# NickDrake117/GNNkeras

Measured on AMD Instinct MI355X. Metric: node-state updates/s (arcs x iterations / s), forward Loop, higher is better.
Workload: dtype f32; 1 GPU; C4 Erdos-Renyi 1000000 nodes / 10000000 arcs, state_dim=64, max_iteration=50, threshold=0 (k=50), node-focused, average aggregation, BN+Dense(159->64,selu) state net

## Files before the change

### gnnkeras_amd/_native.py

```python
from __future__ import annotations

import ctypes as C
import os
import subprocess

import torch

HERE = os.path.dirname(os.path.abspath(__file__))
CSRC = os.path.join(HERE, 'csrc')
LIB_PATH = os.environ.get('GNNKERAS_AMD_LIB') or os.path.join(CSRC, 'libgnnloop.so')

GNN_ABI_VERSION = 10
GNN_MAX_LAYERS = 8
GNN_MAX_TYPES = 8

ACTIVATIONS = {'linear': 0, None: 0, 'relu': 1, 'selu': 2, 'tanh': 3, 'sigmoid': 4, 'elu': 5, 'softplus': 6,
               'softmax': 7}
FOCUS = {'n': 0, 'a': 1, 'g': 2}
FLAG_UNFUSED = 1
FLAG_NO_EARLY_EXIT = 2
FLAG_FUSED_GEN_MASK = 7 << 4
FLAG_TRAIN_HIDDEN_SMALL = 1 << 8
XC_FILL, XC_VALID = 0, 1
FLAG_LDS_HIDDEN = 1 << 9
FLAG_FUSED_GEN2, FLAG_FUSED_GEN4, FLAG_FUSED_GEN5, FLAG_FUSED_GEN6, FLAG_FUSED_GEN7 = 2 << 4, 4 << 4, 5 << 4, 6 << 4, 7 << 4

EXPORTS = ['gnn_last_error', 'gnn_last_status', 'gnn_last_kernel_name', 'gnn_abi_version', 'gnn_struct_size', 'gnn_loop_workspace_bytes', 'gnn_loop_forward', 'gnn_loop_groups_supported', 'gnn_loop_group_max_nodes', 'gnn_aggregate',
           'gnn_loop_xc_applies', 'gnn_loop_route_name', 'gnn_train_xc_applies',
           'gnn_mlp_workspace_bytes', 'gnn_mlp_forward', 'gnn_converged', 'gnn_state_step', 'gnn_state_step_agg', 'gnn_state_ld', 'gnn_debug_occupy', 'gnn_debug_occupy_until', 'gnn_debug_expiry_beacon', 'gnn_debug_host_flag',
           'gnn_debug_f4_tile_plan', 'gnn_debug_f4_tile_queue_const', 'gnn_debug_f4_last_tickets',
           'gnn_device_malloc', 'gnn_device_free', 'gnn_ipc_export', 'gnn_ipc_open', 'gnn_ipc_close', 'gnn_shard_iteration_peers', 'gnn_peer_wait', 'gnn_peer_publish', 'gnn_shard_iteration_split_rows',
           'gnn_shard_setup', 'gnn_shard_iteration', 'gnn_shard_output', 'gnn_gather_rows',
           'gnn_shard_can_split', 'gnn_shard_partial', 'gnn_shard_iteration_split',
           'gnn_dense', 'gnn_fold_bn', 'gnn_dense_grad_workspace_bytes', 'gnn_dense_grad', 'gnn_act_grad',
           'gnn_colstats_workspace_bytes', 'gnn_colstats', 'gnn_first_layer_param_grads', 'gnn_bn_input_grad',
           'gnn_scatter_add_rows', 'gnn_axpby', 'gnn_loss_grad', 'gnn_dropout', 'gnn_adam_step', 'gnn_adam_multi', 'gnn_sgd_step',
           'gnn_converged_gated', 'gnn_aggregate_gated', 'gnn_train_workspace_bytes', 'gnn_train_step', 'gnn_train_groups_supported', 'gnn_ragged_copy',
           'gnn_train_step_ex', 'gnn_train_phases_supported', 'gnn_gate_all',
           'gnn_train_step_composite_ex', 'gnn_train_composite_phases_supported', 'gnn_train_composite_phase_scratch_bytes',
           'gnn_comm_unique_id', 'gnn_comm_create', 'gnn_comm_destroy', 'gnn_shard_loop']
GNN_MAX_SEGMENTS = 6
LOSSES = {'categorical_crossentropy': 0, 'cce': 0, 'binary_crossentropy': 1, 'bce': 1, 'mse': 2,
          'mean_squared_error': 2, 'mae': 3, 'mean_absolute_error': 3}

_f32p = C.POINTER(C.c_float)
# ... 205 lines not shown
        l.gnn_shard_iteration_peers.restype = C.c_int
        l.gnn_shard_iteration_peers.argtypes = [C.POINTER(LoopArgs), C.c_void_p, C.c_void_p, C.c_int32, C.c_void_p, C.c_int32, C.c_int32, C.c_void_p, C.c_int32,
                                                C.POINTER(PeerSet)]
        l.gnn_peer_wait.restype = C.c_int
        l.gnn_peer_wait.argtypes = [C.c_void_p, C.c_int32, C.c_int32, C.c_int32, C.c_void_p, C.c_void_p]
        l.gnn_peer_publish.restype = C.c_int
        l.gnn_peer_publish.argtypes = [C.POINTER(PeerSet), C.c_void_p, C.c_void_p, C.c_int64, C.c_int32, C.c_int32, C.c_int32, C.c_void_p]
        l.gnn_debug_host_flag.restype = C.c_int
        l.gnn_debug_host_flag.argtypes = [C.POINTER(C.POINTER(C.c_int32)), C.POINTER(C.c_void_p)]
        l.gnn_debug_f4_tile_plan.restype = None
        l.gnn_debug_f4_tile_plan.argtypes = [C.c_int32, C.c_int32, C.c_int32, C.POINTER(C.c_int32)]
        l.gnn_debug_f4_tile_queue_const.restype = C.c_int32
        l.gnn_debug_f4_tile_queue_const.argtypes = [C.c_int32, C.c_int32]
        l.gnn_debug_f4_last_tickets.restype = C.c_longlong
        l.gnn_debug_f4_last_tickets.argtypes = []
        l.gnn_debug_expiry_beacon.restype = C.c_int
        l.gnn_debug_expiry_beacon.argtypes = [C.POINTER(C.c_void_p), C.c_int32, C.c_void_p]
        l.gnn_state_step_agg.restype = C.c_int
        l.gnn_state_step_agg.argtypes = [C.POINTER(LoopArgs), C.c_void_p, C.c_void_p, C.c_int32, C.c_void_p, C.c_int32, C.c_void_p, C.c_void_p]
        l.gnn_state_ld.restype = C.c_int32
        l.gnn_state_ld.argtypes = [C.c_int32]
        l.gnn_shard_setup.restype = C.c_int
        l.gnn_shard_setup.argtypes = [C.POINTER(LoopArgs)]
        l.gnn_shard_iteration.restype = C.c_int
        l.gnn_shard_iteration.argtypes = [C.POINTER(LoopArgs), C.c_void_p, C.c_void_p, C.c_int32, C.c_void_p, C.c_int32,
                                          C.c_int32, C.c_void_p, C.c_int32]
        l.gnn_shard_output.restype = C.c_int
        l.gnn_shard_output.argtypes = [C.POINTER(LoopArgs), C.c_void_p, C.c_void_p, C.c_int32]
        vp, i32, f32, sz = C.c_void_p, C.c_int32, C.c_float, C.c_size_t
        protos = {
# ... 88 lines not shown
```

### gnnkeras_amd/csrc/gnnloop.hip

```cpp
#include <hip/hip_runtime.h>
#include <stdarg.h>
#include <stddef.h>
#include <stdio.h>
#include <stdlib.h>
#include <string.h>
#include <algorithm>
#include <mutex>
#include <string>
#include <vector>

#include "../../include/gnnloop.h"
#include "kernels_general.hpp"
#include "kernel_state_fused2.hpp"
#include "kernel_state_fused4.hpp"
#include "kernel_state_small.hpp"
#include "kernel_state_mid.hpp"
#include "kernel_state_lds.hpp"
#include "kernel_state_lds_types.hpp"
#include "kernel_state_wide.hpp"
#include "kernels_batch.hpp"
#include "kernels_setup.hpp"
#include "kernel_rowdense.hpp"
#include "kernel_state_xwide.hpp"

// ... 38 lines not shown
    if (S <= 128) {
        int p = 16;
        while (p < S) p <<= 1;
        return p;
    }
    return round_up(S, 4);
}

struct Knobs {
    int pin;
    int flag_pin, env_pin;
    int mid_max_nodes;
    bool prefix_fusion, xwide, rowdense;
    bool xc; int xc_min_nodes;
    bool tile_queue;
};
const Knobs &process_knobs() {
    static const Knobs once = [] {
        Knobs k = {};
        const char *e;
        k.env_pin = (e = getenv("GNN_FUSED_KERNEL")) ? atoi(e) : 0;
        k.mid_max_nodes = (e = getenv("GNN_MID_MAX_NODES")) ? atoi(e) : 36000;
        k.prefix_fusion = !((e = getenv("GNN_PREFIX_FUSION")) && e[0] == '0');
        k.xwide = !((e = getenv("GNN_XWIDE")) && atoi(e) == 0);
        k.rowdense = !((e = getenv("GNN_ROWDENSE")) && e[0] == '0');
        return k;
    }();
    return once;
}
Knobs knobs(int flags) {
    Knobs k = process_knobs();
    k.flag_pin = (flags & GNN_FLAG_FUSED_GEN_MASK) >> 4;
    k.pin = k.flag_pin ? k.flag_pin : k.env_pin;
    const char *e = getenv("GNN_XC"), *m = getenv("GNN_XC_MIN_NODES");
    k.xc = !(e && atoi(e) == 0);
    k.xc_min_nodes = m ? atoi(m) : 196608;
    const char *q = getenv("GNN_F4_TILE_QUEUE");
    k.tile_queue = !(q && atoi(q) == 0);
    return k;
}

struct Carver {
    char *base;
    size_t off = 0;
    explicit Carver(void *b) : base((char *)b) {}
    template <typename T>
    T *take(size_t count) {
        off = (off + 255) & ~(size_t)255;
        T *p = base ? (T *)(base + off) : nullptr;
        off += count * sizeof(T);
        return p;
    }
};
// ... 334 lines not shown
    float *C; int ldC;
    float *Xc;
    float *Wx;
    bool xc_ok;
    float *buf[2], *agg;
    float *hid[2]; int ld_hid;
    float *Wf_out, *bf_out;
    float *ohid[2]; int ld_ohid;
    float *out_nodes;
    int *idx_src, *idx_dst;
    size_t bytes;
};

constexpr int GNN_SMALL_MAX_TILES = 512;
constexpr int GNN_LOOP_WORDS = 16 + 32 + gnn::MID_BAR_WORDS;
constexpr int GNN_TQ_WORDS = 8;
inline size_t tq_words(const gnn_loop_args_t &a) { return (size_t)GNN_TQ_WORDS * (size_t)a.max_iteration; }

int state_width(const gnn_loop_args_t &a) { return a.state_dim > 0 ? a.state_dim : a.dim_node_label; }

int make_plan(const gnn_loop_args_t &a, void *ws, Plan &p, bool validate_ptrs) {
    memset(&p, 0, sizeof(p));
    if (a.abi_version != GNN_ABI_VERSION) return fail("abi_version %d != %d", a.abi_version, GNN_ABI_VERSION);
    if (a.n_nodes < 0 || a.n_arcs < 0) return fail("negative graph size");
    if (a.state_dim < 0 || a.max_iteration < 0 || !(a.state_threshold >= 0.0f)) return fail("state_dim, max_iteration, state_threshold must be >= 0");
    p.composite = a.composite != 0;
    p.T = p.composite ? a.n_types : 1;
    if (p.T < 1 || p.T > GNN_MAX_TYPES) return fail("n_types %d out of [1,%d]", p.T, GNN_MAX_TYPES);
    if (p.composite && a.max_iteration < 1) return not_covered("composite GNN requires max_iteration > 0");
    p.N = a.n_nodes; p.E = a.n_arcs; p.L = a.dim_node_label; p.A = a.dim_arc_label;
    p.S = state_width(a);
    if (p.S < 1) return fail("state width is 0 (state_dim == 0 and dim_node_label == 0)");
// ... 77 lines not shown
        if (a.n_heavy_segments > 0) {
            if (!a.heavy_seg_beg || !a.heavy_seg_end) return fail("heavy_seg_beg / heavy_seg_end is NULL");
            TRY(check_csr(a.adjacency_light, "adjacency_light", p.N, (a.nodes_src ? a.adjacency.n_src : p.N) + a.n_heavy_segments));
        }
        if (p.composite) {
            if (!a.type_nodes && p.N > 0) return fail("type_nodes is NULL");
            if (a.type_offsets[0] != 0 || a.type_offsets[p.T] != p.N) return fail("type_offsets must span [0, n_nodes]");
            for (int t = 0; t < p.T; ++t)
                TRY(check_csr(a.composite_adjacency[t], "composite_adjacency", p.N, a.nodes_src ? a.adjacency.n_src : p.N));
        }
    }

    Carver c(ws);
    p.flags = c.take<int>(a.max_iteration + GNN_LOOP_WORDS + tq_words(a));
    p.err = p.flags ? p.flags + a.max_iteration + 12 : nullptr;
    p.tq = p.flags ? p.flags + a.max_iteration + GNN_LOOP_WORDS : nullptr;
    p.mid_bar = p.flags ? p.flags + ((a.max_iteration + 16 + 31) & ~31) : nullptr;
    p.pred0 = c.take<int>(std::max(GNN_SMALL_MAX_TILES, p.group_tiles));
    p.d_group_tabs = c.take<int>(a.n_groups > 0 ? 4 * ((size_t)a.n_groups + 1) : 0);
    p.set_bar = c.take<unsigned long long>(a.n_groups > 0 ? 2 * (size_t)a.n_groups : 0);
    for (int t = 0; t < p.T; ++t) {
        p.tp[t].Wf = c.take<float>((size_t)a.net_state[t].in_dim * a.net_state[t].units[0]);
        p.tp[t].bf = c.take<float>(a.net_state[t].units[0]);
    }
    p.Wf_out = c.take<float>((size_t)a.net_output.in_dim * a.net_output.units[0]);
    p.bf_out = c.take<float>(a.net_output.units[0]);
    p.agg_arcs = c.take<float>((size_t)p.N * std::max(p.A, 1));
    p.ld_agg_nodes = p.composite ? sum_dt : (a.state_dim > 0 ? p.L : 0);
    p.agg_nodes = c.take<float>((size_t)p.N * std::max(p.ld_agg_nodes, 1));
    p.ldC = (p.H1max + 3) & ~3;
    p.C = c.take<float>((size_t)p.N * p.ldC);
// ... 202 lines not shown
    sa.nodes_src = a.nodes_src ? a.nodes_src : a.nodes; sa.ld_nodes_src = a.nodes_src ? a.ld_nodes_src : a.ld_nodes;
    sa.adj = gnn::SetupCsr{a.adjacency.rowptr, a.adjacency.src, a.adjacency.w, a.adjacency.row_scale};
    sa.arc_labels = a.arc_labels; sa.ld_arcs = a.ld_arcs; sa.A = p.A;
    sa.arcnode = gnn::SetupCsr{a.arcnode.rowptr, a.arcnode.src, a.arcnode.w, a.arcnode.row_scale};
    if (a.state_dim > 0) { sa.row_nodes = p.S; sa.row_aggn = 2 * p.S + p.L; sa.row_agga = 2 * p.S + 2 * p.L; }
    else                 { sa.row_agga = 2 * p.S; }
    sa.C = p.C; sa.ldC = p.ldC;
    sa.state0 = a.state_dim > 0 ? a.state0 : a.nodes; sa.ld_s0 = a.state_dim > 0 ? p.S : a.ld_nodes;
    sa.S = p.S; sa.thr = a.state_threshold; sa.pred0 = p.pred0;
    sa.zero_a = p.flags; sa.n_a = a.max_iteration + GNN_LOOP_WORDS; sa.zero_b = a.k_out; sa.n_b = std::max(1, p.n_groups);
    gnn::k_setup_small<<<sa.n_tiles + 1, 256, gnn::setup_small_lds(sa.net.H, 2 * L + p.A, std::max(a.net_state[0].in_dim, a.net_output.in_dim)), st>>>(sa);
    LAUNCH_OK();
    return 0;
}

__device__ long long g_f4_last_tickets;
__global__ void k_fold_error(const int *err, float *k_out, const int *tq, int n_tq) {
    long long s = 0;
    for (int i = threadIdx.x; i < n_tq; i += 64) s += tq[i];
    for (int off = 32; off >= 1; off >>= 1) s += __shfl_xor(s, off, 64);
    if (threadIdx.x == 0) {
        g_f4_last_tickets = s;
        if (*err != 0) *k_out = -1.0e9f;
    }
}

int launch_fold_error(const Plan &p, float *k_out, hipStream_t st, const int *tq = nullptr, int n_tq = 0) {
    if (!k_out || !p.err) return 0;
    k_fold_error<<<1, 64, 0, st>>>(p.err, k_out, tq, n_tq);
    LAUNCH_OK();
    return 0;
}

__global__ void k_arc_endpoints(const int *__restrict__ out_index, const int *__restrict__ arc_src,
                                const int *__restrict__ arc_dst, int M, int *__restrict__ idx_src, int *__restrict__ idx_dst) {
    const int m = blockIdx.x * blockDim.x + threadIdx.x;
    if (m < M) { const int e = out_index[m]; idx_src[m] = arc_src[e]; idx_dst[m] = arc_dst[e]; }
}

int output_stage(const gnn_loop_args_t &a, const Plan &p, hipStream_t st) {
    if (p.M == 0) return 0;
    const bool with_labels = !p.composite && a.state_dim > 0;
    MlpRun r;
    r.mlp = &a.net_output; r.Wf = p.Wf_out; r.bf = p.bf_out;
// ... 71 lines not shown
    r.nseg = 1;
    r.segs[0] = gnn::Seg{p.agg, nullptr, p.SP, (int)m.units[1], 0};
    r.M = p.N;
    r.hid[0] = p.hid[0]; r.hid[1] = p.hid[1]; r.ld_hid = p.ld_hid;
    r.Y = dst; r.ldy = p.SP;
    r.gate = gate;
    if (flag_next) { r.pred_old = src; r.ld_pred = p.SP; r.pred_thr = a.state_threshold; r.pred_flag = flag_next; r.pred_k = k_out; r.pred_kval = k_val; }
    TRY(run_mlp(r, st));
    if (flag_next && !r.pred_fused) TRY(launch_converge(gate, dst, src, p.N, p.S, p.SP, p.SP, a.state_threshold, flag_next, k_out, k_val, st));
    return 0;
}

int iteration_fused(const gnn_loop_args_t &a, const Plan &p, IterKernel kernel, const int *gate, int n_gate, int gate_stride,
                    const float *src, float *dst, int row_base, int *flag_next, float *k_out, float k_val,
                    hipStream_t st, const gnn_csr_t *adj_override = nullptr, const float *agg_init = nullptr,
                    const int *rows_override = nullptr, int count_override = 0, const gnn_peer_set_t *peers = nullptr, int *tile_ctr = nullptr) {
    TRY(launch_heavy(a, p, n_gate == 1 ? gate : nullptr, src, st));
    const gnn_csr_t &adj = adj_override ? *adj_override : iter_adjacency(a, p);
    gnn::Fused2Args fa;
    memset(&fa, 0, sizeof(fa));
    fill_fused_args(fa, a, p, adj);
    fa.gate = n_gate ? gate : nullptr; fa.n_gate = n_gate; fa.gate_stride = gate_stride;
    fa.state_in = src; fa.state_out = dst; fa.row_base = row_base; fa.err = p.err;
    if (rows_override && fa.n_types == 1) {
        fa.tp[0].rows = rows_override; fa.tp[0].count = count_override;
        if (count_override == 0) fa.n_types = 0;
    }
    fa.flag_next = flag_next;
    fa.k_out = k_out; fa.k_val = k_val;
    fa.agg_init = agg_init;
    if (peers) {
        if (peers->n_peers < 0 || peers->n_peers > GNN_MAX_PEERS) return fail("n_peers %d out of [0, %d]", peers->n_peers, GNN_MAX_PEERS);
        fa.n_peers = peers->n_peers;
        for (int i = 0; i < peers->n_peers; ++i) fa.peer_out[i] = peers->state_out_full[i];
    }
    if (p.xc_ok && !adj.w && (agg_init || size_generation(p, a.flags) == 4)) fa.Xc = p.Xc;
    if (tile_ctr && kernel == IterKernel::fused4 && p.T == 1 && fa.n_types == 1 && !rows_override && !agg_init && !peers) fa.tq_ctr = tile_ctr;
    if (fa.n_types == 0) {
        if (k_out) TRY(launch_converge(fa.gate, src, src, 0, p.S, p.SP, p.SP, a.state_threshold, flag_next, k_out, k_val, st));
        return 0;
    }
    if (fa.n_peers > 0 && (p.SP == 128 || p.T != 1 || adj.w || a.net_state[0].n_layers != 1 || (p.SP != 32 && p.SP != 64) || p.n_heavy != 0))
        return fail("peer stores: homogeneous one-layer shards without per-arc weights or hub rows, state widths 17 .. 64");
    if (kernel == IterKernel::wide) FUSED_OK(gnn::launch_wide(fa, device_cus(), st, 0));
    else if (kernel == IterKernel::fused4 || agg_init || fa.n_peers > 0) FUSED_OK(gnn::launch_fused4(fa, p.SP, device_cus(), st));
    else FUSED_OK(gnn::launch_fused2(fa, p.SP, 8, device_cus(), st));
    return 0;
}

int loop_whole(const gnn_loop_args_t &a, const Plan &p, bool mid, const float *first, float *const B[2], const int *pred0,
               int n_pred0, float *state_final, hipStream_t st) {
    gnn::SmallArgs sa;
// ... 261 lines not shown
    if (first == a.state0 && a.state_out != a.state0 && (reinterpret_cast<uintptr_t>(a.state_out) & 15) == 0 && a.max_iteration > 0)
        B[a.max_iteration & 1] = a.state_out;
    if (a.ev_loop_begin) HIP_OK(hipEventRecord((hipEvent_t)a.ev_loop_begin, st));
    int persistent = 2;
    if (route.whole == WholeLoop::small) {
        persistent = loop_whole(a, p, false, first, B, small_setup ? p.pred0 : nullptr, small_setup ? p.group_tiles : 0, a.state_out, st);
        if (persistent == 1) return 1;
        if (persistent == 2 && small_setup) return fail("whole-loop kernel refused a graph its set-up kernel accepted");
    }
    bool loop_done = persistent == 0;
    if (!loop_done && route.try_mid) {
        const int rc = loop_whole(a, p, true, first, B, nullptr, 0, nullptr, st);
        if (rc == 1) return 1;
        loop_done = rc == 0;
    }
    int *const tq = (!small_setup && knobs(a.flags).tile_queue) ? p.tq : nullptr;
    for (int it = 0; !loop_done && it < a.max_iteration; ++it) {
        const int *gate = no_exit ? nullptr : p.flags + it;
        const float *src = it == 0 ? first : B[it & 1];
        float *dst = B[(it + 1) & 1];
        if (route.iter.fused())                  TRY(iteration_fused(a, p, kernel, gate, gate ? 1 : 0, 0, src, dst, 0, p.flags + it + 1, a.k_out, (float)(it + 1), st,
                                                                     nullptr, nullptr, nullptr, 0, nullptr, tq ? tq + (size_t)GNN_TQ_WORDS * it : nullptr));
        else if (kernel == IterKernel::prefix)   TRY(iteration_prefix(a, p, gate, src, dst, p.flags + it + 1, a.k_out, (float)(it + 1), st));
        else if (kernel == IterKernel::xwide)    TRY(iteration_xwide(a, p, gate, src, dst, p.flags + it + 1, a.k_out, (float)(it + 1), st));
        else                                     TRY(iteration_unfused(a, p, gate, src, dst, 0, p.flags + it + 1, a.k_out, (float)(it + 1), st));
    }

    if (a.ev_loop_end) HIP_OK(hipEventRecord((hipEvent_t)a.ev_loop_end, st));

    if (persistent != 0) {
        const long total = (long)p.N * p.S;
        if (total > 0) {
            gnn::k_select_state<<<std::min(cdiv(total, 256), 256 * 16), 256, 0, st>>>(a.k_out, first, B[0], B[1], p.SP, a.state_out, p.S, p.N, p.S);
            LAUNCH_OK();
        }
    }
    TRY(output_stage(a, p, st));
    if (!loop_done && (route.iter.fused() || kernel == IterKernel::xwide) && a.max_iteration > 0)
        TRY(launch_fold_error(p, a.k_out, st, tq, tq ? (int)tq_words(a) : 0));
    return 0;
}

int gnn_loop_groups_supported(const gnn_loop_args_t *args) {
    if (!args || args->n_groups < 1) return 0;
    Plan p;
    if (make_plan(*args, nullptr, p, false)) return 0;
    const LoopRoute route = route_loop(*args, p);
    if (route.whole == WholeLoop::lds || route.whole == WholeLoop::lds_types) return 2;
    if (p.composite || args->n_groups > GNN_MAX_GROUPS) return 0;
    return route.whole == WholeLoop::small && route.small_setup ? 1 : 0;
}

int gnn_loop_group_max_nodes(const gnn_loop_args_t *args) {
    if (!args) return 0;
// ... 120 lines not shown
    int polls = 0;
    while (wall_clock64() - t0 < ticks) {
        if (release && __hip_atomic_load(release, __ATOMIC_RELAXED, __HIP_MEMORY_SCOPE_SYSTEM) != 0) break;
        __builtin_amdgcn_s_sleep(64); ++polls;
    }
    if (threadIdx.x == 0 && polls < 0) { occ_smem[0] = polls; *sink = occ_smem[0]; }
}

void gnn_debug_f4_tile_plan(int32_t ntiles, int32_t n_workgroups, int32_t ahead, int32_t *out56) {
    for (int xcd = 0; xcd < 8; ++xcd) {
        const gnn::F4TilePlan q = gnn::f4_tile_plan(ntiles, n_workgroups, xcd, ahead);
        int32_t *o = out56 + 7 * xcd;
        o[0] = q.t_begin; o[1] = q.t_end; o[2] = q.blk; o[3] = q.T1; o[4] = q.pool_begin; o[5] = q.pool_end; o[6] = q.n_chunks;
    }
}
int32_t gnn_debug_f4_tile_queue_const(int32_t which, int32_t padded_width) {
    switch (which) {
        case 0: return gnn::F4_TQ_CH;
        case 1: return padded_width == 64 ? gnn::Fused4Cfg<64>::AHEAD : padded_width == 32 ? gnn::Fused4Cfg<32>::AHEAD : padded_width == 16 ? gnn::Fused4Cfg<16>::AHEAD : -1;
        case 2: return gnn::F4_TQ_MIN_SHARE;
        case 3: return gnn::F4_TQ_MAX_CHUNKS;
        case 4: return gnn::F4_TQ_TAB;
        default: return -1;
    }
}
long long gnn_debug_f4_last_tickets(void) {
    long long v = -1;
    if (hipDeviceSynchronize() != hipSuccess) return -1;
    return hipMemcpyFromSymbol(&v, HIP_SYMBOL(g_f4_last_tickets), sizeof(v)) == hipSuccess ? v : -1;
}
// ... 292 lines not shown
```

### gnnkeras_amd/csrc/kernel_state_fused2.hpp

```cpp
#pragma once
#include <hip/hip_runtime.h>
#include "kernels_general.hpp"

namespace gnn {

struct FusedType {
    const int *rows;
    int count;
    const float *Wf;
    int wrow_state, wrow_agg;
    int H, act;
    const float *W2;
    const float *b2;
    int act2;
    const float *Wc;
    int out2;
};

struct Fused2Args {
    const int *gate; int n_gate, gate_stride;
    const int *rowptr, *src;
    const float *w, *row_scale;
    const float *state_in;
    float *state_out;
    int row_base;
    const float *C; int ldC;
    int n_types;
    FusedType tp[GNN_MAX_TYPES];
    int blk_begin[GNN_MAX_TYPES + 1];
    int S;
    float thr;
    int *flag_next;
    float *k_out; float k_val;
    int *err;
    int *tq_ctr;
    const float *Xc;
    const float *agg_init;
    const void *hdr; void *hdr_write;
    float *peer_out[GNN_MAX_PEERS]; int n_peers;
};

inline char *last_kernel_name() { static thread_local char name[96] = ""; return name; }
#define GNN_SET_KERNEL_NAME(...) snprintf(::gnn::last_kernel_name(), 96, __VA_ARGS__)

template <int SP, int TM, int NW>
struct Fused2Cfg {
    static constexpr int NT = 64 * NW;
    static constexpr int LPR = SP / 4;
    static constexpr int NPP = NT / LPR;
    static constexpr int NPASS = TM / NPP;
// ... 323 lines not shown
```

### gnnkeras_amd/csrc/kernel_state_fused4.hpp

```cpp
#pragma once
#include <hip/hip_runtime.h>
#include "kernel_state_fused2.hpp"
#include "buffer_ops.hpp"

namespace gnn {

constexpr int XC_K = 32;

constexpr int F4_TQ_CH = 2;
constexpr int F4_TQ_NUM = 7, F4_TQ_DEN = 8;
constexpr int F4_TQ_TAB = 1024;
constexpr int F4_TQ_MAX_CHUNKS = 960;
constexpr int F4_TQ_MIN_SHARE = 16;
constexpr int F4_TQ_END = -2;
struct F4TilePlan { int t_begin, t_end, blk, T1, pool_begin, pool_end, n_chunks; };
__host__ __device__ inline F4TilePlan f4_tile_plan(int ntiles, int nblk, int xcd, int ahead) {
    F4TilePlan q;
    const int tpx = (ntiles + 7) >> 3;
    q.blk = (nblk + 7 - xcd) >> 3;
    q.t_begin = xcd * tpx < ntiles ? xcd * tpx : ntiles;
    q.t_end = (xcd + 1) * tpx < ntiles ? (xcd + 1) * tpx : ntiles;
    const int n = q.t_end - q.t_begin, b = q.blk > 0 ? q.blk : 1;
    const int n_min = ntiles - 7 * tpx > 0 ? ntiles - 7 * tpx : 0, b_max = (nblk + 7) >> 3;
    const bool queue = (nblk & 7) == 0 && nblk > 0 && n_min >= F4_TQ_MIN_SHARE * b_max && (int)((long)F4_TQ_NUM * n_min / ((long)F4_TQ_DEN * b_max)) >= ahead;
    if (!queue) {
        q.T1 = (n + b - 1) / b; q.pool_begin = q.pool_end = q.t_end; q.n_chunks = 0;
        return q;
    }
    q.T1 = (int)((long)F4_TQ_NUM * n / ((long)F4_TQ_DEN * b));
    if (n - q.T1 * b > F4_TQ_MAX_CHUNKS * F4_TQ_CH) q.T1 = (n - F4_TQ_MAX_CHUNKS * F4_TQ_CH + b - 1) / b;
    q.pool_begin = q.t_begin + q.T1 * b; q.pool_end = q.t_end;
    q.n_chunks = (q.pool_end - q.pool_begin + F4_TQ_CH - 1) / F4_TQ_CH;
    return q;
}

template <int SP, int NC = 4, bool L2 = false, bool XC = false, int VPL = 1, bool TQ = false>
struct Fused4Cfg {
    static constexpr int NW = 16, NT = 64 * NW;
    static constexpr int NCONS = NC;
    static constexpr int NPROD = NW - NCONS;
    static constexpr int LPR = SP / (4 * VPL);
    static constexpr int RPWV = 64 / LPR;
    static constexpr int PPT = 16 / RPWV;
    static constexpr int IPL = 16 / LPR;
    static constexpr int LDX = 2 * SP + 2;
    static constexpr bool SWZ = SP >= 32;
    static constexpr int LDW = SWZ ? SP : SP + 32;
    static constexpr int NCT = SP / 16;
    static constexpr int NS = SP == 64 ? (L2 ? 3 : (XC ? 4 : 5)) : 8;
    static constexpr int WROWS = 2 * SP + (XC ? XC_K : 0);
    static constexpr int SLOT = 16 * LDX;
    static constexpr int W2F = L2 ? SP * LDW + SP : 0;
    static constexpr int AHEAD = (2 * NPROD + PPT - 1) / PPT + F4_TQ_CH + 2;
    static constexpr size_t LDS_BYTES = sizeof(float) * ((size_t)NS * SLOT + WROWS * LDW + W2F) + sizeof(int) * (2 * NS + (TQ ? F4_TQ_TAB : 0));
};

__device__ __forceinline__ void activate4(int act, f32x4 &x) {
#define F4_ALL(expr)                                        \
    _Pragma("unroll") for (int e = 0; e < 4; ++e) {         \
        const float v = x[e];                               \
        x[e] = (expr);                                      \
    }
    switch (act) {
        case GNN_ACT_RELU: F4_ALL(fmaxf(v, 0.0f)) break;
        case GNN_ACT_SELU: F4_ALL(v > 0.0f ? 1.0507009873554805f * v : (1.0507009873554805f * 1.6732632423543772f) * (expf(v) - 1.0f)) break;
        case GNN_ACT_TANH: F4_ALL(tanhf(v)) break;
        case GNN_ACT_SIGMOID: F4_ALL(1.0f / (1.0f + expf(-v))) break;
        case GNN_ACT_ELU: F4_ALL(v > 0.0f ? v : expf(v) - 1.0f) break;
        case GNN_ACT_SOFTPLUS: F4_ALL(v > 20.0f ? v : log1pf(expf(v))) break;
// ... 44 lines not shown
    const int tid = threadIdx.x, lane = tid & 63, wave = tid >> 6;
    if (tid == 0) F4_STAMP(0);
    const int S = a.S;
    int ty = 0;
    while (ty + 1 < a.n_types && (int)blockIdx.x >= a.blk_begin[ty + 1]) ++ty;
    const FusedType tp = a.tp[ty];
    const int O2 = tp.out2 > 0 ? tp.out2 : S;
    const int bid = blockIdx.x - a.blk_begin[ty], nblk = a.blk_begin[ty + 1] - a.blk_begin[ty];
    const int count = tp.count;
    const int *__restrict__ rows = tp.rows;

    const int ntiles = (count + 15) / 16;
    const int xcd = bid & 7, lb = bid >> 3;
    const int blk_per_xcd = (nblk + 7 - xcd) >> 3;
    const int tpx = (ntiles + 7) >> 3;
    const int t_end = min(ntiles, (xcd + 1) * tpx);
    const int t_first = xcd * tpx + lb;
    const int T = t_first < t_end ? (t_end - t_first + blk_per_xcd - 1) / blk_per_xcd : 0;
    const F4TilePlan tq = TQ ? f4_tile_plan(ntiles, nblk, xcd, Cfg::AHEAD) : F4TilePlan{};
    int tq_end = F4_TQ_TAB;
    auto tq_entry = [&](int ci) -> int {
        if (ci >= tq_end) return F4_TQ_END;
        int v, spin = 0;
        while ((v = __builtin_amdgcn_readfirstlane(f4_ld_acquire(&tab[ci]))) == 0) {
            if (spin >= SPIN_MAX) { bad = 1; v = F4_TQ_END; break; }
            ++spin; __builtin_amdgcn_s_sleep(1);
        }
        if (v == F4_TQ_END) tq_end = ci;
        return v;
    };
    auto tile_of = [&](int L) -> int {
        if constexpr (!TQ) return L < T ? t_first + L * blk_per_xcd : F4_TQ_END;
        else {
            if (L < tq.T1) return t_first + L * blk_per_xcd;
// ... 87 lines not shown
        }
        Ws[k * LDW + (Cfg::SWZ ? (n ^ ((k & 1) << 4)) : n)] = v;
    }
    if (L2) {
        for (int i = tid; i < SP * SP; i += NT) {
            const int k = i / SP, n = i % SP;
            W2s[k * LDW + (Cfg::SWZ ? (n ^ ((k & 1) << 4)) : n)] = (k < tp.H && n < O2) ? tp.W2[(size_t)k * O2 + n] : 0.0f;
        }
        if (tid < SP) W2s[SP * LDW + tid] = tid < O2 ? tp.b2[tid] : 0.0f;
    }
    if (tid < 2 * NS) fill[tid] = 0;
    if constexpr (TQ) for (int i = tid; i < F4_TQ_TAB; i += NT) tab[i] = 0;
    __syncthreads();
    if (!open) return;
    if (tid == 0) F4_STAMP(1);

    if (wave >= Cfg::NCONS) {
#ifdef GNN_F4_PROFILE
        const unsigned long long tr_ = f4_now();
#endif
        for (int n = p; TQ ? tlA != F4_TQ_END : n < njobs; n += Cfg::NPROD) {
            const int t = n / Cfg::PPT;
            const int row = (n % Cfg::PPT) * Cfg::RPWV + qr;
            const int j = jA;
            bool draws = false;
            int dci = 0, dprev = 1, ticket = 0;
            if constexpr (TQ) {
                const int x = t + Cfg::AHEAD - tq.T1;
                draws = n % Cfg::PPT == 0 && x >= 0 && x % F4_TQ_CH == 0;
                if (draws) {
// ... 105 lines not shown
                *reinterpret_cast<float2 *>(xr + SP) = make_float2(acc[x][0], acc[x][1]);
                *reinterpret_cast<float2 *>(xr + SP + 2) = make_float2(acc[x][2], acc[x][3]);
            }
            if (l4 == 0) Xs[s * Cfg::SLOT + row * LDX + 2 * SP] = __int_as_float(j);
            if (lane == 0) __hip_atomic_fetch_add(&fill[s], 1, __ATOMIC_RELEASE, __HIP_MEMORY_SCOPE_WORKGROUP);
            if (n == p && p == 0 && lane == 0) F4_STAMP(2);
        }
#ifdef GNN_F4_PROFILE
        if (lane == 0) atomicAdd(&g_f4_prof[6], f4_now() - tr_);
#endif
    } else {
        const int r = lane & 15, g = lane >> 4;
#ifdef GNN_F4_PROFILE
        const unsigned long long tr_ = f4_now();
#endif
        for (int t = wave; TQ || t < T; t += Cfg::NCONS) {
            int tl = 0;
            if constexpr (TQ) {
                tl = tile_of(t);
                if (tl == F4_TQ_END) break;
            }
            f32x4 c[Cfg::NCT];
            float xa[XC ? XC_K / 4 : 1];
            if (XC) {
                const int m = TQ ? (tl >= 0 ? tl * 16 + r : count) : (t_first + t * blk_per_xcd) * 16 + r;
                const int jr = buf_ld_i32(r_rows, m < count ? 4u * (unsigned)m : BUF_OFF);
                const int jx = m < count ? (rows ? jr : m) : -1;
#pragma unroll
                for (int q = 0; q < XC_K / 4; ++q)
                    xa[q] = buf_ld_f32(r_C, jx >= 0 ? ((unsigned)jx * (unsigned)XC_K + (unsigned)(4 * q + g)) * 4u : BUF_OFF);
// ... 162 lines not shown
#endif
            if (lane == 0) __hip_atomic_store(&freed[s], round + 1, __ATOMIC_RELEASE, __HIP_MEMORY_SCOPE_WORKGROUP);
        }
#ifdef GNN_F4_PROFILE
        if (lane == 0) atomicAdd(&g_f4_prof[7], f4_now() - tr_);
#endif
    }

    any = __syncthreads_or(any);
    bad = __syncthreads_or(bad);
    if (tid == 0) F4_STAMP(3);
    if (tid == 0) {
        if (any && a.flag_next) atomicOr(a.flag_next, 1);
        if (bad && a.err) atomicOr(a.err, 1);
        if (blockIdx.x == 0 && a.k_out) *a.k_out = a.k_val;
    }
}

inline int fused4_blocks(int ntiles, long total_tiles, int budget) {
    if (ntiles <= 0) return 0;
    const int nb = (int)std::min<long>((ntiles + 3) / 4, std::max<long>(8, budget * (long)ntiles / std::max<long>(total_tiles, 1)));
    return std::max(8, nb / 8 * 8);
}

template <int SP, bool HAS_W, int DEPTH, bool L2 = false, int NC = 4, bool INIT = false, bool XC = false, int VPL = 1, bool HDR = false, bool PEERS = false, bool TQ = false>
int launch_fused4_one(Fused2Args &fa, int n_cu, hipStream_t st) {
    using Cfg = Fused4Cfg<SP, NC, L2, XC, VPL, TQ>;
    static_assert(2 * Cfg::LDS_BYTES <= 160 * 1024, "two workgroups per CU");
    static bool attr = false;
    if (!attr) {
// ... 74 lines not shown
```

### include/gnnloop.h

```cpp
#ifndef GNNLOOP_H
#define GNNLOOP_H

#include <stddef.h>
#include <stdint.h>

#ifdef __cplusplus
extern "C" {
#endif

#define GNN_ABI_VERSION 10

enum gnn_activation {
    GNN_ACT_LINEAR = 0, GNN_ACT_RELU = 1, GNN_ACT_SELU = 2, GNN_ACT_TANH = 3, GNN_ACT_SIGMOID = 4,
    GNN_ACT_ELU = 5, GNN_ACT_SOFTPLUS = 6, GNN_ACT_SOFTMAX = 7
};

enum gnn_focus { GNN_FOCUS_NODE = 0, GNN_FOCUS_ARC = 1, GNN_FOCUS_GRAPH = 2 };

enum gnn_flags {
    GNN_FLAG_UNFUSED = 1,
    GNN_FLAG_NO_EARLY_EXIT = 2,
    GNN_FLAG_FUSED_GEN2 = 2 << 4, GNN_FLAG_FUSED_GEN4 = 4 << 4,
    GNN_FLAG_FUSED_GEN5 = 5 << 4, GNN_FLAG_FUSED_GEN6 = 6 << 4, GNN_FLAG_FUSED_GEN7 = 7 << 4, GNN_FLAG_FUSED_GEN_MASK = 7 << 4,
    GNN_FLAG_TRAIN_HIDDEN_SMALL = 1 << 8,
// ... 103 lines not shown
int gnn_converged(const float *state, const float *state_old, int32_t n, int32_t dim, int32_t ld, float threshold,
                  int32_t *flag, void *stream);

int gnn_state_step(const gnn_loop_args_t *args, const float *state_in, float *state_out, int32_t *flag_out);

int gnn_state_step_agg(const gnn_loop_args_t *args, const float *state_in, const float *aggregated_nodes, int32_t ld_aggregated_nodes,
                       const float *aggregated_arcs, int32_t ld_aggregated_arcs, float *state_out, int32_t *flag_out);

int gnn_debug_occupy(int32_t n_workgroups, int32_t lds_bytes, int32_t milliseconds, void *stream);
int gnn_debug_occupy_until(int32_t n_workgroups, int32_t lds_bytes, int32_t max_milliseconds, const int32_t *release_flag, void *stream);
int gnn_debug_host_flag(int32_t **host_out, int32_t **dev_out);
int gnn_debug_expiry_beacon(int32_t **beacon_out, int32_t reset, void *stream);
void gnn_debug_f4_tile_plan(int32_t ntiles, int32_t n_workgroups, int32_t ahead, int32_t *out56);
int32_t gnn_debug_f4_tile_queue_const(int32_t which, int32_t padded_width);
long long gnn_debug_f4_last_tickets(void);

int32_t gnn_state_ld(int32_t state_width);
int gnn_gather_rows(const float *src, int32_t ld_src, const int32_t *idx, int32_t M, int32_t width, float *dst,
                    int32_t ld_dst, void *stream);
int gnn_shard_setup(const gnn_loop_args_t *args);
int gnn_shard_iteration(const gnn_loop_args_t *args, const float *state_in_full, float *state_out_full,
                        int32_t row_base, const int32_t *gate, int32_t n_gate, int32_t gate_stride, int32_t *flag_out,
                        int32_t iteration);
int gnn_shard_output(const gnn_loop_args_t *args, const float *buf0_full, const float *buf1_full, int32_t row_base);
int gnn_shard_can_split(const gnn_loop_args_t *args);
int gnn_shard_partial(const gnn_loop_args_t *args, const gnn_csr_t *adjacency_own, const float *state_in_full,
                      float *agg_partial);
int gnn_shard_iteration_split(const gnn_loop_args_t *args, const gnn_csr_t *adjacency_halo, const float *agg_partial,
                              const float *state_in_full, float *state_out_full, int32_t row_base, const int32_t *gate,
                              int32_t n_gate, int32_t gate_stride, int32_t *flag_out, int32_t iteration);
// ... 209 lines not shown
```

Measured before the change: 22.08 billion arc-updates/s.

## Rebalance fused4 tile ranges across XCDs using measured per-XCD finish times

Adds a per-iteration feedback loop to the fused4 tile queue. Each workgroup records per-XCD start and exit wall-clock stamps into the tile-queue row, and block 0 of the next iteration turns these into new per-XCD tile bounds, moving tiles toward faster XCDs with damping. The aim is to cut tail time when some XCDs finish their static tile share late. The cost is extra atomics, a larger LDS footprint, a serial rebalance computation in one thread, and possible oscillation or noise from wall-clock based decisions.

```diff
diff --git a/gnnkeras_amd/_native.py b/gnnkeras_amd/_native.py
--- a/gnnkeras_amd/_native.py
+++ b/gnnkeras_amd/_native.py
@@ -29,6 +29,7 @@
            'gnn_loop_xc_applies', 'gnn_loop_route_name', 'gnn_train_xc_applies',
            'gnn_mlp_workspace_bytes', 'gnn_mlp_forward', 'gnn_converged', 'gnn_state_step', 'gnn_state_step_agg', 'gnn_state_ld', 'gnn_debug_occupy', 'gnn_debug_occupy_until', 'gnn_debug_expiry_beacon', 'gnn_debug_host_flag',
            'gnn_debug_f4_tile_plan', 'gnn_debug_f4_tile_queue_const', 'gnn_debug_f4_last_tickets',
+           'gnn_debug_f4_tile_plan_bounds', 'gnn_debug_f4_rebalance', 'gnn_debug_f4_bounds_from_shares', 'gnn_debug_f4_xcd_times',
            'gnn_device_malloc', 'gnn_device_free', 'gnn_ipc_export', 'gnn_ipc_open', 'gnn_ipc_close', 'gnn_shard_iteration_peers', 'gnn_peer_wait', 'gnn_peer_publish', 'gnn_shard_iteration_split_rows',
            'gnn_shard_setup', 'gnn_shard_iteration', 'gnn_shard_output', 'gnn_gather_rows',
            'gnn_shard_can_split', 'gnn_shard_partial', 'gnn_shard_iteration_split',
@@ -264,6 +265,14 @@
         l.gnn_debug_f4_tile_queue_const.argtypes = [C.c_int32, C.c_int32]
         l.gnn_debug_f4_last_tickets.restype = C.c_longlong
         l.gnn_debug_f4_last_tickets.argtypes = []
+        l.gnn_debug_f4_tile_plan_bounds.restype = None
+        l.gnn_debug_f4_tile_plan_bounds.argtypes = [C.c_int32, C.c_int32, C.c_int32, C.POINTER(C.c_int32), C.POINTER(C.c_int32)]
+        l.gnn_debug_f4_rebalance.restype = C.c_int32
+        l.gnn_debug_f4_rebalance.argtypes = [C.c_int32, C.c_int32, C.POINTER(C.c_int32), C.POINTER(C.c_uint64), C.POINTER(C.c_int32)]
+        l.gnn_debug_f4_bounds_from_shares.restype = C.c_int32
+        l.gnn_debug_f4_bounds_from_shares.argtypes = [C.c_int32, C.c_int32, C.POINTER(C.c_int32), C.POINTER(C.c_int32)]
+        l.gnn_debug_f4_xcd_times.restype = C.c_int32
+        l.gnn_debug_f4_xcd_times.argtypes = [C.c_int32, C.POINTER(C.c_int32), C.POINTER(C.c_int64), C.POINTER(C.c_int32)]
         l.gnn_debug_expiry_beacon.restype = C.c_int
         l.gnn_debug_expiry_beacon.argtypes = [C.POINTER(C.c_void_p), C.c_int32, C.c_void_p]
         l.gnn_state_step_agg.restype = C.c_int
diff --git a/gnnkeras_amd/csrc/gnnloop.hip b/gnnkeras_amd/csrc/gnnloop.hip
--- a/gnnkeras_amd/csrc/gnnloop.hip
+++ b/gnnkeras_amd/csrc/gnnloop.hip
@@ -76,6 +76,7 @@
     bool prefix_fusion, xwide, rowdense;
     bool xc; int xc_min_nodes;
     bool tile_queue;
+    bool xcd_balance, xcd_shares; int xcd_share[8];
 };
 const Knobs &process_knobs() {
     static const Knobs once = [] {
@@ -99,6 +100,20 @@
     k.xc_min_nodes = m ? atoi(m) : 196608;
     const char *q = getenv("GNN_F4_TILE_QUEUE");
     k.tile_queue = !(q && atoi(q) == 0);
+    const char *b = getenv("GNN_F4_XCD_BALANCE"), *s = getenv("GNN_F4_XCD_SHARES");
+    k.xcd_balance = !(b && atoi(b) == 0);
+    k.xcd_shares = false;
+    if (s && k.xcd_balance) {
+        int n = 0;
+        for (const char *c = s; n < 8; ++n) {
+            char *end;
+            const long v = strtol(c, &end, 10);
+            if (end == c || v < 0 || v > 1000000) break;
+            k.xcd_share[n] = (int)v;
+            c = *end == ',' ? end + 1 : end;
+        }
+        k.xcd_shares = n == 8;
+    }
     return k;
 }
 
@@ -463,8 +478,8 @@
 
 constexpr int GNN_SMALL_MAX_TILES = 512;
 constexpr int GNN_LOOP_WORDS = 16 + 32 + gnn::MID_BAR_WORDS;
-constexpr int GNN_TQ_WORDS = 8;
-inline size_t tq_words(const gnn_loop_args_t &a) { return (size_t)GNN_TQ_WORDS * (size_t)a.max_iteration; }
+constexpr int GNN_TQ_WORDS = gnn::F4_TQ_ROW;
+inline size_t tq_words(const gnn_loop_args_t &a) { return 2 + (size_t)GNN_TQ_WORDS * (size_t)a.max_iteration; }
 
 int state_width(const gnn_loop_args_t &a) { return a.state_dim > 0 ? a.state_dim : a.dim_node_label; }
 
@@ -572,7 +587,7 @@
     Carver c(ws);
     p.flags = c.take<int>(a.max_iteration + GNN_LOOP_WORDS + tq_words(a));
     p.err = p.flags ? p.flags + a.max_iteration + 12 : nullptr;
-    p.tq = p.flags ? p.flags + a.max_iteration + GNN_LOOP_WORDS : nullptr;
+    p.tq = p.flags ? p.flags + ((a.max_iteration + GNN_LOOP_WORDS + 1) & ~1) : nullptr;
     p.mid_bar = p.flags ? p.flags + ((a.max_iteration + 16 + 31) & ~31) : nullptr;
     p.pred0 = c.take<int>(std::max(GNN_SMALL_MAX_TILES, p.group_tiles));
     p.d_group_tabs = c.take<int>(a.n_groups > 0 ? 4 * ((size_t)a.n_groups + 1) : 0);
@@ -805,20 +820,32 @@
     return 0;
 }
 
+constexpr int GNN_F4_DBG_ROWS = 64;
 __device__ long long g_f4_last_tickets;
-__global__ void k_fold_error(const int *err, float *k_out, const int *tq, int n_tq) {
+__device__ int g_f4_last_rows[GNN_F4_DBG_ROWS * GNN_TQ_WORDS + 1];
+__global__ void k_fold_error(const int *err, float *k_out, const int *tq, int n_rows) {
     long long s = 0;
-    for (int i = threadIdx.x; i < n_tq; i += 64) s += tq[i];
+    for (int i = threadIdx.x; i < 8 * n_rows; i += 64) s += tq[(i >> 3) * GNN_TQ_WORDS + (i & 7)];
     for (int off = 32; off >= 1; off >>= 1) s += __shfl_xor(s, off, 64);
+    const int keep = n_rows < GNN_F4_DBG_ROWS ? n_rows : GNN_F4_DBG_ROWS;
+    for (int i = threadIdx.x; i < keep * GNN_TQ_WORDS; i += 64) g_f4_last_rows[1 + i] = tq[i];
     if (threadIdx.x == 0) {
+        g_f4_last_rows[0] = keep;
         g_f4_last_tickets = s;
         if (*err != 0) *k_out = -1.0e9f;
     }
 }
 
-int launch_fold_error(const Plan &p, float *k_out, hipStream_t st, const int *tq = nullptr, int n_tq = 0) {
+struct TileBounds { int b[9]; };
+__global__ void k_tq_preset(int *tq, int n_rows, TileBounds tb) {
+    const int r = blockIdx.x * blockDim.x + threadIdx.x;
+    if (r < n_rows)
+        for (int x = 0; x < 9; ++x) tq[(size_t)r * GNN_TQ_WORDS + gnn::F4_TQ_ROW_BOUNDS + x] = tb.b[x];
+}
+
+int launch_fold_error(const Plan &p, float *k_out, hipStream_t st, const int *tq = nullptr, int n_rows = 0) {
     if (!k_out || !p.err) return 0;
-    k_fold_error<<<1, 64, 0, st>>>(p.err, k_out, tq, n_tq);
+    k_fold_error<<<1, 64, 0, st>>>(p.err, k_out, tq, n_rows);
     LAUNCH_OK();
     return 0;
 }
@@ -920,7 +947,8 @@
 int iteration_fused(const gnn_loop_args_t &a, const Plan &p, IterKernel kernel, const int *gate, int n_gate, int gate_stride,
                     const float *src, float *dst, int row_base, int *flag_next, float *k_out, float k_val,
                     hipStream_t st, const gnn_csr_t *adj_override = nullptr, const float *agg_init = nullptr,
-                    const int *rows_override = nullptr, int count_override = 0, const gnn_peer_set_t *peers = nullptr, int *tile_ctr = nullptr) {
+                    const int *rows_override = nullptr, int count_override = 0, const gnn_peer_set_t *peers = nullptr, int *tile_ctr = nullptr,
+                    int tile_next_off = 0) {
     TRY(launch_heavy(a, p, n_gate == 1 ? gate : nullptr, src, st));
     const gnn_csr_t &adj = adj_override ? *adj_override : iter_adjacency(a, p);
     gnn::Fused2Args fa;
@@ -941,7 +969,7 @@
         for (int i = 0; i < peers->n_peers; ++i) fa.peer_out[i] = peers->state_out_full[i];
     }
     if (p.xc_ok && !adj.w && (agg_init || size_generation(p, a.flags) == 4)) fa.Xc = p.Xc;
-    if (tile_ctr && kernel == IterKernel::fused4 && p.T == 1 && fa.n_types == 1 && !rows_override && !agg_init && !peers) fa.tq_ctr = tile_ctr;
+    if (tile_ctr && kernel == IterKernel::fused4 && p.T == 1 && fa.n_types == 1 && !rows_override && !agg_init && !peers) { fa.tq_ctr = tile_ctr; fa.tq_next_off = tile_next_off; }
     if (fa.n_types == 0) {
         if (k_out) TRY(launch_converge(fa.gate, src, src, 0, p.S, p.SP, p.SP, a.state_threshold, flag_next, k_out, k_val, st));
         return 0;
@@ -1233,13 +1261,24 @@
         if (rc == 1) return 1;
         loop_done = rc == 0;
     }
-    int *const tq = (!small_setup && knobs(a.flags).tile_queue) ? p.tq : nullptr;
+    const Knobs kn = knobs(a.flags);
+    int *const tq = (!small_setup && kn.tile_queue) ? p.tq : nullptr;
+    if (tq && !loop_done && kn.xcd_shares && route.iter.fused() && kernel == IterKernel::fused4 && p.T == 1 && a.max_iteration > 0) {
+        const int ntiles = (p.tp[0].count + 15) / 16;
+        TileBounds tb;
+        if (gnn::f4_bounds_from_shares(ntiles, gnn::fused4_blocks(ntiles, ntiles, 2 * device_cus()), kn.xcd_share, tb.b)) {
+            k_tq_preset<<<cdiv(a.max_iteration, 64), 64, 0, st>>>(tq, a.max_iteration, tb);
+            LAUNCH_OK();
+        }
+    }
+    const bool tq_feed = kn.xcd_balance && !kn.xcd_shares;
     for (int it = 0; !loop_done && it < a.max_iteration; ++it) {
         const int *gate = no_exit ? nullptr : p.flags + it;
         const float *src = it == 0 ? first : B[it & 1];
         float *dst = B[(it + 1) & 1];
         if (route.iter.fused())                  TRY(iteration_fused(a, p, kernel, gate, gate ? 1 : 0, 0, src, dst, 0, p.flags + it + 1, a.k_out, (float)(it + 1), st,
-                                                                     nullptr, nullptr, nullptr, 0, nullptr, tq ? tq + (size_t)GNN_TQ_WORDS * it : nullptr));
+                                                                     nullptr, nullptr, nullptr, 0, nullptr, tq ? tq + (size_t)GNN_TQ_WORDS * it : nullptr,
+                                                                     tq_feed && it >= 1 && it + 1 < a.max_iteration ? GNN_TQ_WORDS : 0));
         else if (kernel == IterKernel::prefix)   TRY(iteration_prefix(a, p, gate, src, dst, p.flags + it + 1, a.k_out, (float)(it + 1), st));
         else if (kernel == IterKernel::xwide)    TRY(iteration_xwide(a, p, gate, src, dst, p.flags + it + 1, a.k_out, (float)(it + 1), st));
         else                                     TRY(iteration_unfused(a, p, gate, src, dst, 0, p.flags + it + 1, a.k_out, (float)(it + 1), st));
@@ -1256,7 +1295,7 @@
     }
     TRY(output_stage(a, p, st));
     if (!loop_done && (route.iter.fused() || kernel == IterKernel::xwide) && a.max_iteration > 0)
-        TRY(launch_fold_error(p, a.k_out, st, tq, tq ? (int)tq_words(a) : 0));
+        TRY(launch_fold_error(p, a.k_out, st, tq, tq ? a.max_iteration : 0));
     return 0;
 }
 
@@ -1407,6 +1446,43 @@
         o[0] = q.t_begin; o[1] = q.t_end; o[2] = q.blk; o[3] = q.T1; o[4] = q.pool_begin; o[5] = q.pool_end; o[6] = q.n_chunks;
     }
 }
+void gnn_debug_f4_tile_plan_bounds(int32_t ntiles, int32_t n_workgroups, int32_t ahead, const int32_t *bounds9, int32_t *out56) {
+    for (int xcd = 0; xcd < 8; ++xcd) {
+        const gnn::F4TilePlan q = gnn::f4_tile_plan(ntiles, n_workgroups, xcd, ahead, bounds9 ? bounds9[xcd] : 0, bounds9 ? bounds9[xcd + 1] : 0);
+        int32_t *o = out56 + 7 * xcd;
+        o[0] = q.t_begin; o[1] = q.t_end; o[2] = q.blk; o[3] = q.T1; o[4] = q.pool_begin; o[5] = q.pool_end; o[6] = q.n_chunks;
+    }
+}
+int32_t gnn_debug_f4_rebalance(int32_t ntiles, int32_t n_workgroups, const int32_t *bounds_in9, const uint64_t *ticks8, int32_t *bounds_out9) {
+    gnn::F4Balance wk;
+    for (int x = 0; x < 8; ++x) wk.ticks[x] = ticks8[x];
+    for (int x = 0; x < 9; ++x) wk.bounds_in[x] = bounds_in9 ? bounds_in9[x] : 0;
+    const bool q = gnn::f4_rebalance(ntiles, n_workgroups, wk);
+    for (int x = 0; x < 9; ++x) bounds_out9[x] = wk.bounds_out[x];
+    return q ? 1 : 0;
+}
+int32_t gnn_debug_f4_bounds_from_shares(int32_t ntiles, int32_t n_workgroups, const int32_t *shares8, int32_t *bounds_out9) {
+    int sh[8], bout[9];
+    for (int x = 0; x < 8; ++x) sh[x] = shares8[x];
+    const bool q = gnn::f4_bounds_from_shares(ntiles, n_workgroups, sh, bout);
+    for (int x = 0; x < 9; ++x) bounds_out9[x] = bout[x];
+    return q ? 1 : 0;
+}
+int32_t gnn_debug_f4_xcd_times(int32_t max_rows, int32_t *bounds, int64_t *ticks, int32_t *exits) {
+    static int host[GNN_F4_DBG_ROWS * GNN_TQ_WORDS + 1];
+    if (hipDeviceSynchronize() != hipSuccess) return -1;
+    if (hipMemcpyFromSymbol(host, HIP_SYMBOL(g_f4_last_rows), sizeof(host)) != hipSuccess) return -1;
+    const int n = std::min(host[0], (int)max_rows);
+    for (int r = 0; r < n; ++r) {
+        const int *row = host + 1 + r * GNN_TQ_WORDS;
+        unsigned long long w[9];
+        memcpy(w, row + gnn::F4_TQ_ROW_EXIT, sizeof(w));
+        for (int x = 0; x < 9; ++x) bounds[9 * r + x] = row[gnn::F4_TQ_ROW_BOUNDS + x];
+        for (int x = 0; x < 8; ++x) ticks[8 * r + x] = (w[8] != 0 && w[x] != 0) ? (int64_t)(w[x] - ~w[8]) : 0;
+        exits[r] = row[gnn::F4_TQ_ROW_COUNT];
+    }
+    return n;
+}
 int32_t gnn_debug_f4_tile_queue_const(int32_t which, int32_t padded_width) {
     switch (which) {
         case 0: return gnn::F4_TQ_CH;
diff --git a/gnnkeras_amd/csrc/kernel_state_fused2.hpp b/gnnkeras_amd/csrc/kernel_state_fused2.hpp
--- a/gnnkeras_amd/csrc/kernel_state_fused2.hpp
+++ b/gnnkeras_amd/csrc/kernel_state_fused2.hpp
@@ -34,6 +34,7 @@
     float *k_out; float k_val;
     int *err;
     int *tq_ctr;
+    int tq_next_off;
     const float *Xc;
     const float *agg_init;
     const void *hdr; void *hdr_write;
diff --git a/gnnkeras_amd/csrc/kernel_state_fused4.hpp b/gnnkeras_amd/csrc/kernel_state_fused4.hpp
--- a/gnnkeras_amd/csrc/kernel_state_fused4.hpp
+++ b/gnnkeras_amd/csrc/kernel_state_fused4.hpp
@@ -14,7 +14,8 @@
 constexpr int F4_TQ_MIN_SHARE = 16;
 constexpr int F4_TQ_END = -2;
 struct F4TilePlan { int t_begin, t_end, blk, T1, pool_begin, pool_end, n_chunks; };
-__host__ __device__ inline F4TilePlan f4_tile_plan(int ntiles, int nblk, int xcd, int ahead) {
+constexpr int F4_TQ_ROW = 40, F4_TQ_ROW_BOUNDS = 8, F4_TQ_ROW_COUNT = 17, F4_TQ_ROW_EXIT = 18, F4_TQ_ROW_START = 34;
+__host__ __device__ inline F4TilePlan f4_tile_plan(int ntiles, int nblk, int xcd, int ahead, int rb = 0, int re = 0) {
     F4TilePlan q;
     const int tpx = (ntiles + 7) >> 3;
     q.blk = (nblk + 7 - xcd) >> 3;
@@ -29,9 +30,105 @@
     }
     q.T1 = (int)((long)F4_TQ_NUM * n / ((long)F4_TQ_DEN * b));
     if (n - q.T1 * b > F4_TQ_MAX_CHUNKS * F4_TQ_CH) q.T1 = (n - F4_TQ_MAX_CHUNKS * F4_TQ_CH + b - 1) / b;
+    if (re > 0) { q.t_begin = rb; q.t_end = re; }
     q.pool_begin = q.t_begin + q.T1 * b; q.pool_end = q.t_end;
     q.n_chunks = (q.pool_end - q.pool_begin + F4_TQ_CH - 1) / F4_TQ_CH;
     return q;
+}
+
+constexpr int F4_BAL_NUM = 3, F4_BAL_DEN = 4;
+struct F4Balance {
+    int bounds_in[9], bounds_out[9];
+    unsigned long long ticks[8];
+    long long want[8];
+    unsigned long long s[8];
+    int n_in[8], eq[9], lo[8], hi[8], d[8];
+};
+__host__ __device__ inline bool f4_bounds_from_targets(int ntiles, int nblk, F4Balance &wk) {
+    bool queue = true;
+    long long sum = 0;
+#pragma unroll 1
+    for (int x = 0; x < 8; ++x) {
+        const F4TilePlan q = f4_tile_plan(ntiles, nblk, x, 0);
+        wk.eq[x] = q.t_begin; wk.eq[x + 1] = q.t_end;
+        queue = queue && q.n_chunks > 0;
+        const int half = (q.pool_end - q.pool_begin) / (2 * F4_TQ_CH), room = F4_TQ_MAX_CHUNKS - q.n_chunks;
+        const int lo = -half, hi = half < room ? half : room;
+        long long w = wk.want[x] - (q.t_end - q.t_begin);
+        w = (w + (w < 0 ? -(F4_TQ_CH / 2) : F4_TQ_CH / 2)) / F4_TQ_CH;
+        w = w < lo ? lo : (w > hi ? hi : w);
+        wk.lo[x] = lo; wk.hi[x] = hi; wk.d[x] = (int)w;
+        sum += w;
+    }
+#pragma unroll 1
+    for (int pass = 0; pass < 8 && sum != 0; ++pass) {
+        int open_ = 0;
+#pragma unroll 1
+        for (int x = 0; x < 8; ++x) open_ += sum > 0 ? wk.d[x] > wk.lo[x] : wk.d[x] < wk.hi[x];
+        open_ = open_ > 0 ? open_ : 1;
+        const long long per = ((sum < 0 ? -sum : sum) + open_ - 1) / open_;
+#pragma unroll 1
+        for (int x = 0; x < 8; ++x) {
+            const int d = wk.d[x];
+            if (sum > 0) { long long t = d - wk.lo[x]; t = t < per ? t : per; t = t < sum ? t : sum; wk.d[x] = d - (int)t; sum -= t; }
+            else if (sum < 0) { long long t = wk.hi[x] - d; t = t < per ? t : per; t = t < -sum ? t : -sum; wk.d[x] = d + (int)t; sum += t; }
+        }
+    }
+    int acc = 0;
+    wk.bounds_out[0] = wk.eq[0];
+#pragma unroll 1
+    for (int x = 0; x < 8; ++x) {
+        acc += queue ? wk.d[x] : 0;
+        wk.bounds_out[x + 1] = wk.eq[x + 1] + (x < 7 ? F4_TQ_CH * acc : 0);
+    }
+    return queue;
+}
+__host__ __device__ inline bool f4_bounds_from_shares(int ntiles, int nblk, const int share[8], int out[9]) {
+    F4Balance wk;
+    long long tot = 0;
+    bool ok = true;
+    for (int x = 0; x < 8; ++x) { tot += share[x]; ok = ok && share[x] >= 0 && share[x] <= 1000000; }
+    for (int x = 0; x < 8; ++x) {
+        const F4TilePlan q = f4_tile_plan(ntiles, nblk, x, 0);
+        wk.want[x] = q.t_end - q.t_begin + (ok && tot > 0 ? (long long)ntiles * (8ll * share[x] - tot) / (8 * tot) : 0);
+    }
+    const bool queue = f4_bounds_from_targets(ntiles, nblk, wk);
+    for (int x = 0; x < 9; ++x) out[x] = wk.bounds_out[x];
+    return queue;
+}
+__host__ __device__ inline bool f4_rebalance(int ntiles, int nblk, F4Balance &wk) {
+    unsigned long long tmax = 0, smax = 0, ssum = 0;
+    bool sane = wk.bounds_in[0] == 0 && wk.bounds_in[8] == ntiles, same = true, measured = true;
+#pragma unroll 1
+    for (int x = 0; x < 8; ++x) {
+        sane = sane && wk.bounds_in[x + 1] >= wk.bounds_in[x];
+        tmax = wk.ticks[x] > tmax ? wk.ticks[x] : tmax;
+        same = same && wk.ticks[x] == wk.ticks[0];
+        measured = measured && wk.ticks[x] != 0;
+    }
+    measured = measured && !same && tmax < (1ull << 31);
+    const int tpx = (ntiles + 7) >> 3;
+#pragma unroll 1
+    for (int x = 0; x < 8; ++x) {
+        const int e0 = x * tpx < ntiles ? x * tpx : ntiles, e1 = (x + 1) * tpx < ntiles ? (x + 1) * tpx : ntiles;
+        const int n = sane ? wk.bounds_in[x + 1] - wk.bounds_in[x] : e1 - e0;
+        wk.n_in[x] = n;
+        const unsigned long long s = measured ? ((unsigned long long)n << 28) / wk.ticks[x] : 0;
+        wk.s[x] = s;
+        smax = s > smax ? s : smax;
+    }
+    int sh = 0;
+    while ((smax >> sh) >= (1ull << 28)) ++sh;
+#pragma unroll 1
+    for (int x = 0; x < 8; ++x) ssum += wk.s[x] >> sh;
+    measured = measured && ssum > 0;
+#pragma unroll 1
+    for (int x = 0; x < 8; ++x) {
+        const long long n = wk.n_in[x];
+        const long long fair = measured ? (long long)((unsigned long long)ntiles * (wk.s[x] >> sh) / ssum) : n;
+        wk.want[x] = n + (fair - n) * F4_BAL_NUM / F4_BAL_DEN;
+    }
+    return f4_bounds_from_targets(ntiles, nblk, wk);
 }
 
 template <int SP, int NC = 4, bool L2 = false, bool XC = false, int VPL = 1, bool TQ = false>
@@ -52,7 +149,7 @@
     static constexpr int SLOT = 16 * LDX;
     static constexpr int W2F = L2 ? SP * LDW + SP : 0;
     static constexpr int AHEAD = (2 * NPROD + PPT - 1) / PPT + F4_TQ_CH + 2;
-    static constexpr size_t LDS_BYTES = sizeof(float) * ((size_t)NS * SLOT + WROWS * LDW + W2F) + sizeof(int) * (2 * NS + (TQ ? F4_TQ_TAB : 0));
+    static constexpr size_t LDS_BYTES = sizeof(float) * ((size_t)NS * SLOT + WROWS * LDW + W2F) + sizeof(int) * (2 * NS + (TQ ? F4_TQ_TAB : 0)) + (TQ ? (sizeof(F4Balance) + 15) / 16 * 16 : 0);
 };
 
 __device__ __forceinline__ void activate4(int act, f32x4 &x) {
@@ -127,10 +224,12 @@
     const int xcd = bid & 7, lb = bid >> 3;
     const int blk_per_xcd = (nblk + 7 - xcd) >> 3;
     const int tpx = (ntiles + 7) >> 3;
-    const int t_end = min(ntiles, (xcd + 1) * tpx);
-    const int t_first = xcd * tpx + lb;
+    int tq_rb = 0, tq_re = 0;
+    if constexpr (TQ) { tq_rb = a.tq_ctr[F4_TQ_ROW_BOUNDS + xcd]; tq_re = a.tq_ctr[F4_TQ_ROW_BOUNDS + xcd + 1]; }
+    const F4TilePlan tq = TQ ? f4_tile_plan(ntiles, nblk, xcd, Cfg::AHEAD, tq_rb, tq_re) : F4TilePlan{};
+    const int t_end = TQ ? tq.t_end : min(ntiles, (xcd + 1) * tpx);
+    const int t_first = (TQ ? tq.t_begin : xcd * tpx) + lb;
     const int T = t_first < t_end ? (t_end - t_first + blk_per_xcd - 1) / blk_per_xcd : 0;
-    const F4TilePlan tq = TQ ? f4_tile_plan(ntiles, nblk, xcd, Cfg::AHEAD) : F4TilePlan{};
     int tq_end = F4_TQ_TAB;
     auto tq_entry = [&](int ci) -> int {
         if (ci >= tq_end) return F4_TQ_END;
@@ -248,6 +347,9 @@
     __syncthreads();
     if (!open) return;
     if (tid == 0) F4_STAMP(1);
+    if constexpr (TQ) {
+        if (tid == 0 && lb == 0) atomicMax(reinterpret_cast<unsigned long long *>(a.tq_ctr + F4_TQ_ROW_START), ~wall_clock64());
+    }
 
     if (wave >= Cfg::NCONS) {
 #ifdef GNN_F4_PROFILE
@@ -383,6 +485,20 @@
 #ifdef GNN_F4_PROFILE
         const unsigned long long tr_ = f4_now();
 #endif
+        if (TQ && blockIdx.x == 0 && tid == 0 && a.tq_next_off != 0) {
+            F4Balance &wk = *reinterpret_cast<F4Balance *>(tab + F4_TQ_TAB);
+            const int *prev = a.tq_ctr - a.tq_next_off;
+            const unsigned long long *stamp = reinterpret_cast<const unsigned long long *>(prev + F4_TQ_ROW_EXIT);
+            const unsigned long long t0c = stamp[8];
+#pragma unroll 1
+            for (int x = 0; x < 9; ++x) {
+                wk.bounds_in[x] = prev[F4_TQ_ROW_BOUNDS + x];
+                if (x < 8) wk.ticks[x] = stamp[x] != 0 && t0c != 0 ? stamp[x] - ~t0c : 0;
+            }
+            f4_rebalance((a.tp[0].count + 15) / 16, a.blk_begin[1] - a.blk_begin[0], wk);
+#pragma unroll 1
+            for (int x = 0; x < 9; ++x) a.tq_ctr[a.tq_next_off + F4_TQ_ROW_BOUNDS + x] = wk.bounds_out[x];
+        }
         for (int t = wave; TQ || t < T; t += Cfg::NCONS) {
             int tl = 0;
             if constexpr (TQ) {
@@ -575,6 +691,12 @@
         if (any && a.flag_next) atomicOr(a.flag_next, 1);
         if (bad && a.err) atomicOr(a.err, 1);
         if (blockIdx.x == 0 && a.k_out) *a.k_out = a.k_val;
+    }
+    if constexpr (TQ) {
+        if (tid == 0) {
+            atomicMax(reinterpret_cast<unsigned long long *>(a.tq_ctr + F4_TQ_ROW_EXIT) + xcd, wall_clock64());
+            atomicAdd(a.tq_ctr + F4_TQ_ROW_COUNT, 1);
+        }
     }
 }
 
diff --git a/include/gnnloop.h b/include/gnnloop.h
--- a/include/gnnloop.h
+++ b/include/gnnloop.h
@@ -141,6 +141,10 @@
 void gnn_debug_f4_tile_plan(int32_t ntiles, int32_t n_workgroups, int32_t ahead, int32_t *out56);
 int32_t gnn_debug_f4_tile_queue_const(int32_t which, int32_t padded_width);
 long long gnn_debug_f4_last_tickets(void);
+void gnn_debug_f4_tile_plan_bounds(int32_t ntiles, int32_t n_workgroups, int32_t ahead, const int32_t *bounds9, int32_t *out56);
+int32_t gnn_debug_f4_rebalance(int32_t ntiles, int32_t n_workgroups, const int32_t *bounds_in9, const uint64_t *ticks8, int32_t *bounds_out9);
+int32_t gnn_debug_f4_bounds_from_shares(int32_t ntiles, int32_t n_workgroups, const int32_t *shares8, int32_t *bounds_out9);
+int32_t gnn_debug_f4_xcd_times(int32_t max_rows, int32_t *bounds, int64_t *ticks, int32_t *exits);
 
 int32_t gnn_state_ld(int32_t state_width);
 int gnn_gather_rows(const float *src, int32_t ld_src, const int32_t *idx, int32_t M, int32_t width, float *dst,
```

Result: no change. 22.25 billion arc-updates/s, median of 6 (+0.7%).
